# VincentStimper/normalizing-flows

Hardware: AMD Instinct MI355X
Metric: samples/sec + NLL (nats/dim), 32-layer RQ-NSF d=64 B=65536 (higher is better)
Workload: dtype f32; 1 GPU; BASELINE configs[1]: log_prob of 32 x [CoupledRQS(d=64, 2 blocks, 128 hidden, K=8, tail 3) + LULinearPermute(64)] + DiagGaussian, batch 65536 rows/GPU, N(0,I) inputs, sigma=0.01 perturbed seeded weights; rows_per_gpu=65536, global_rows=65536, layers=32, launch=hipGraph replay, parallelism=dp1

## Files before the change

include/nf_mi355x.h:

```cpp
#ifndef NF_MI355X_H
#define NF_MI355X_H

#include <stdint.h>

#ifdef __cplusplus
extern "C" {
#endif

typedef void *nf_stream_t;

enum { NF_OK = 0, NF_EIO = -5, NF_EFAULT = -14, NF_EINVAL = -22, NF_ERANGE = -34, NF_ENOTSUP = -95 };
enum { NF_F32 = 0, NF_F64 = 1 };
enum { NF_LD_WRITE = 0, NF_LD_ADD = 1, NF_LD_SUB = -1 };
enum { NF_TAILS_NONE = 0, NF_TAILS_LINEAR = 1, NF_TAILS_CIRCULAR = 2, NF_TAILS_FEATURE = 3  };
enum { NF_SCALE_EXP = 0, NF_SCALE_SIGMOID = 1, NF_SCALE_SIGMOID_INV = 2, NF_SCALE_NONE = 3 };
enum { NF_RQS_DENSITY = 0, NF_RQS_SAMPLE_IDENTITY = 1, NF_RQS_SAMPLE_TRANSFORM = 2 };

const char *nf_version(void);
const char *nf_strerror(int code);
int nf_mfma_clock_probe(void *out2_u64, void *sink_f32, int iters, nf_stream_t stream);
int nf_max_bins(void);
int nf_persistent_workgroups(void);

int nf_rqs_spline(const void *x, const void *w, int64_t ldw, const void *h, int64_t ldh, const void *d,
// ... 22 lines not shown
                        const int64_t *transform_idx, int nT, int64_t B, int D, int K, int tails,
                        double tail_bound, double min_bin_width, double min_bin_height, double min_derivative,
                        double wh_div, int mode, void *grad_x, void *grad_cond, void *grad_uw, void *grad_uh,
                        void *grad_ud, int dtype, nf_stream_t stream);

int nf_rqs_coupling_bwd_ft(const void *x, const void *grad_y, const void *grad_logdet, const void *cond,
                           const void *uw, const void *uh, const void *ud, const int64_t *identity_idx, int nI,
                           const int64_t *transform_idx, int nT, int64_t B, int D, int K, int tails,
                           double tail_bound, double min_bin_width, double min_bin_height, double min_derivative,
                           double wh_div, int mode, void *grad_x, void *grad_cond, void *grad_uw, void *grad_uh,
                           void *grad_ud, int dtype, const int32_t *tails_t, const void *bound_t,
                           const int32_t *tails_i, const void *bound_i, nf_stream_t stream);

int nf_rqs_coupling_bwd_ft_wave_fits(int nI, int nT);
int nf_rqs_coupling_bwd_ft_wave(const void *x, const void *grad_y, const void *grad_logdet, const void *cond,
                                const void *uw, const void *uh, const void *ud, const int64_t *identity_idx, int nI,
                                const int64_t *transform_idx, int nT, int64_t B, int D, int K, int tails,
                                double tail_bound, double min_bin_width, double min_bin_height, double min_derivative,
                                double wh_div, int mode, void *grad_x, void *grad_cond, void *grad_uw, void *grad_uh,
                                void *grad_ud, int dtype, const int32_t *tails_t, const void *bound_t,
                                const int32_t *tails_i, const void *bound_i, nf_stream_t stream);

int nf_rqs_fused_final_row(int K, int g, int rb, int rho);
int64_t nf_rqs_fused_pack_size(int nI, int nT, int hidden, int num_blocks, int K);
int nf_rqs_fused_pack(void *wpack, const void *w_init, const void *b_init, const void *const *w_blocks,
                      const void *const *b_blocks, const void *w_final, const void *b_final, const void *uw,
                      const void *uh, const void *ud, int nI, int nT, int hidden, int num_blocks, int K,
                      double tail_bound, double min_bin_width, double min_bin_height, double min_derivative,
                      nf_stream_t stream);
int nf_rqs_fused_pack_lu(void *wpack, int num_blocks, const int64_t *perm, const void *lower_entries,
                         const void *upper_entries, const void *unconstrained_upper_diag, const void *bias, int D,
                         double eps, int K, nf_stream_t stream);
int nf_rqs_fused(const void *x, void *y, void *logdet, const void *wpack, int mask_parity, int fuse_lu, int64_t B,
                 int D, int hidden, int num_blocks, int K, double tail_bound, double min_bin_width,
                 double min_bin_height, double min_derivative, int direction, int acc, nf_stream_t stream);
int nf_rqs_fused_chain(const void *x, void *y, void *logdet, const void *const *wpacks, const int *mask_parities,
                       int num_layers, int fuse_lu, int64_t B, int D, int hidden, int num_blocks, int K,
                       double tail_bound, double min_bin_width, double min_bin_height, double min_derivative,
                       int direction, int acc, nf_stream_t stream);
int nf_rqs_fused_small_batch(int enable);

int nf_rqs_fused_pack_final(void *wpack, const void *w_final, const void *b_final, const void *uw, const void *uh,
                            const void *ud, int hidden, int num_blocks, int K, double tail_bound, double min_bin_width,
                            double min_bin_height, double min_derivative, nf_stream_t stream);
int nf_rqs_fused_train_fwd(const void *x, const void *h2, void *y, void *logdet, void *cond_out, const void *wpack,
                           int mask_parity, int64_t B, int D, int hidden, int num_blocks, int K, double tail_bound,
// ... 333 lines not shown
```

normalizing-flows_amd/csrc/fused_common.hpp:

```cpp
#pragma once
#include "common.hpp"

namespace nf {

constexpr int F_MAX_LAYERS = 64;

typedef float f32x16 __attribute__((ext_vector_type(16)));
typedef float f32x4 __attribute__((ext_vector_type(4)));

constexpr int F_D = 64;
constexpr int F_NI = 32;
constexpr int F_H = 128;
constexpr int F_K = 8;
constexpr int F_M = 3 * F_K - 1;
constexpr int F_STAGE = 4096;
constexpr int F_TABW = 3 * (F_K + 1);
constexpr int F_HDR = 64;

struct FusedLayout {
    int nblk;
    int K = F_K;
    __host__ __device__ int ngroups() const { return K; }
    __host__ __device__ int nfinal() const { return 3 * K; }
    __host__ __device__ int tabw() const { return 3 * (K + 1); }
    __host__ __device__ int bias_final_floats() const { return 96 * K; }
    __host__ __device__ int small_floats() const { return 128 + 256 * nblk + bias_final_floats() + F_NI * tabw() + 128; }
    __host__ __device__ int off_bias_init() const { return 0; }
    __host__ __device__ int off_bias_hidden(int lin) const { return 128 + 128 * lin; }
    __host__ __device__ int off_bias_final() const { return 128 + 256 * nblk; }
    __host__ __device__ int off_tables() const { return off_bias_final() + bias_final_floats(); }
    __host__ __device__ int off_bias_lu(int dir) const { return off_tables() + F_NI * tabw() + 64 * dir; }
    __host__ __device__ int lu_stage(int dir) const { return 1 + 8 * nblk + nfinal() + dir; }
    __host__ __device__ int small_padded() const { return (small_floats() + 1023) / 1024 * 1024; }
    __host__ __device__ int off_stages() const { return F_HDR + small_padded(); }
    __host__ __device__ int nstages(bool lu) const { return 1 + 8 * nblk + nfinal() + (lu ? 1 : 0); }
    __host__ __device__ int64_t total_floats() const { return (int64_t)off_stages() + (int64_t)(nstages(false) + 2) * F_STAGE; }
};

template <int KB>
__host__ __device__ inline int final_row_k(int g, int rb, int rho) {
    constexpr int MP = 3 * KB, M = 3 * KB - 1, FPL = 16 / KB, GQ = KB / 4;
    const int q = rho >> 3, hh = (rho >> 2) & 1, r = rho & 3;
    const int v = 16 * rb + 4 * q + r;
    const int f = v / MP, prm = v % MP;
    if (prm >= M) return -1;
    const int tf = 8 * (g / GQ) + 4 * hh + (g % GQ) * FPL + f;
    return tf * M + prm;
}
__host__ __device__ inline int final_row(int g, int rb, int rho) { return final_row_k<F_K>(g, rb, rho); }

__host__ __device__ inline int final_bwd_row(int g, int v, int hq) {
    return v >= F_M ? -1 : (8 * (g >> 1) + 4 * (hq >> 1) + 2 * (g & 1) + (hq & 1)) * F_M + v;
}

__host__ __device__ inline int lu_out_col(int m, int rho) {
    const int q = rho >> 3, hh = (rho >> 2) & 1, r = rho & 3;
    return 16 * (2 * m + (q >> 1)) + 8 * hh + 4 * (q & 1) + r;
}
__host__ __device__ inline int lu_in_col(int s, int hk, int r4) { return 16 * (s >> 1) + 8 * hk + 4 * (s & 1) + r4; }

__device__ __forceinline__ float fexp(float x) { return __builtin_amdgcn_exp2f(x * 1.44269504088896340736f); }
__device__ __forceinline__ float flog(float x) { return __builtin_amdgcn_logf(x) * 0.69314718055994530942f; }
__device__ __forceinline__ float frcp(float x) { return __builtin_amdgcn_rcpf(x); }
__device__ __forceinline__ float fsqrt(float x) { return __builtin_amdgcn_sqrtf(x); }
__device__ __forceinline__ float fsoftplus(float x) {
    const float t = fexp(fminf(x, 20.0f));
    const float u = 1.0f + t;
    const float w = u - 1.0f;
    const float l1p = (w == 0.0f) ? t : flog(u) * (t * frcp(w));
    return x > 20.0f ? x : l1p;
}

// ... 68 lines not shown
    }
    float dl0 = p.edge_logit, dl1 = p.edge_logit;
#pragma unroll
    for (int k = 0; k < KB - 1; ++k) {
        dl0 = (bin == k + 1) ? prm[2 * KB + k] : dl0;
        dl1 = (bin == k) ? prm[2 * KB + k] : dl1;
    }
    const float d0 = p.min_d + fsoftplus(dl0), d1 = p.min_d + fsoftplus(dl1);
    float yy, ll;
    if (!INVERSE)
        rqs_eval_bin_fast<false>(x, slo, shi - slo, olo, ohi - olo, d0, d1, yy, ll);
    else
        rqs_eval_bin_fast<true>(x, olo, ohi - olo, slo, shi - slo, d0, d1, yy, ll);
    y = inside ? yy : x;
    lad = inside ? ll : 0.0f;
}

typedef float f32x2e __attribute__((ext_vector_type(2)));
typedef int i32x2e __attribute__((ext_vector_type(2)));
__device__ __forceinline__ f32x2e pk_fma(f32x2e a, f32x2e b, f32x2e c) { return __builtin_elementwise_fma(a, b, c); }
__device__ __forceinline__ f32x2e pk_rcp(f32x2e a) { return f32x2e{frcp(a[0]), frcp(a[1])}; }
__device__ __forceinline__ f32x2e pk_log(f32x2e a) { return f32x2e{flog(a[0]), flog(a[1])}; }
__device__ __forceinline__ f32x2e pk_bc(float a) { return f32x2e{a, a}; }

template <int N>
__device__ __forceinline__ void rqs_descend2(f32x2e x, const f32x2e (&s)[N + 1], const f32x2e (&o)[N + 1], const f32x2e (&d)[N + 1],
                                             f32x2e &slo, f32x2e &shi, f32x2e &olo, f32x2e &ohi, f32x2e &dl0, f32x2e &dl1) {
    if constexpr (N == 1) {
        slo = s[0]; shi = s[1]; olo = o[0]; ohi = o[1]; dl0 = d[0]; dl1 = d[1];
    } else {
        constexpr int H = N / 2;
        const i32x2e c = x >= s[H];
        f32x2e s2[H + 1], o2[H + 1], d2[H + 1];
#pragma unroll
        for (int i = 0; i <= H; ++i) {
            s2[i] = c ? s[H + i] : s[i];
            o2[i] = c ? o[H + i] : o[i];
            d2[i] = c ? d[H + i] : d[i];
        }
        rqs_descend2<H>(x, s2, o2, d2, slo, shi, olo, ohi, dl0, dl1);
    }
}

template <bool INVERSE>
__device__ __forceinline__ void rqs_eval_bin_fast2(f32x2e x, f32x2e cw, f32x2e bw, f32x2e ch, f32x2e bh, f32x2e d0, f32x2e d1,
                                                   f32x2e &y, f32x2e &lad) {
    const f32x2e delta = bh * pk_rcp(bw);
    const f32x2e dsum = d0 + d1 - 2.0f * delta;
    f32x2e theta, den;
    if (!INVERSE) {
        theta = (x - cw) * pk_rcp(bw);
        const f32x2e t1mt = theta * (1.0f - theta);
        const f32x2e num = bh * (delta * theta * theta + d0 * t1mt);
        den = delta + dsum * t1mt;
        y = ch + num * pk_rcp(den);
    } else {
        const f32x2e dy = x - ch;
        const f32x2e a = dy * dsum + bh * (delta - d0);
        const f32x2e b = bh * d0 - dy * dsum;
        const f32x2e c = -delta * dy;
        const f32x2e disc = b * b - 4.0f * a * c;
        theta = (2.0f * c) * pk_rcp(-b - f32x2e{fsqrt(disc[0]), fsqrt(disc[1])});
        y = theta * bw + cw;
        den = delta + dsum * (theta * (1.0f - theta));
    }
    const f32x2e omt = 1.0f - theta;
    const f32x2e dnum = delta * delta * (d1 * theta * theta + 2.0f * delta * (theta * omt) + d0 * omt * omt);
    const f32x2e l = pk_log(dnum) - 2.0f * pk_log(den);
    lad = INVERSE ? -l : l;
}

template <bool INVERSE, int KB = F_K>
__device__ __forceinline__ void rqs_regs2(const RqsParams<float> &p, float x0, float x1, const float (&prm0)[3 * KB],
                                          const float (&prm1)[3 * KB], float &y0, float &y1, float &lad0, float &lad1) {
    static_assert((KB & (KB - 1)) == 0, "binary descent");
    const f32x2e x = {x0, x1};
    const i32x2e inside = (x >= p.left) & (x <= p.right);
    f32x2e mw = {prm0[0], prm1[0]}, mh = {prm0[KB], prm1[KB]};
#pragma unroll
    for (int k = 1; k < KB; ++k) {
        mw = f32x2e{fmaxf(mw[0], prm0[k]), fmaxf(mw[1], prm1[k])};
        mh = f32x2e{fmaxf(mh[0], prm0[KB + k]), fmaxf(mh[1], prm1[KB + k])};
    }
    f32x2e pw[KB], ph[KB];
#pragma unroll
    for (int k = 0; k < KB; ++k) {
        const f32x2e aw = f32x2e{prm0[k], prm1[k]} - mw, ah = f32x2e{prm0[KB + k], prm1[KB + k]} - mh;
        const f32x2e ew = {__builtin_amdgcn_exp2f(aw[0]), __builtin_amdgcn_exp2f(aw[1])};
        const f32x2e eh = {__builtin_amdgcn_exp2f(ah[0]), __builtin_amdgcn_exp2f(ah[1])};
        pw[k] = k == 0 ? ew : pw[k - 1] + ew;
        ph[k] = k == 0 ? eh : ph[k - 1] + eh;
    }
    const f32x2e cw = ((p.right - p.left) * p.scale_w) * pk_rcp(pw[KB - 1]);
    const f32x2e ch = ((p.top - p.bottom) * p.scale_h) * pk_rcp(ph[KB - 1]);
    f32x2e kw[KB + 1], kh[KB + 1], dp[KB + 1];
    kw[0] = pk_bc(p.left);
    kh[0] = pk_bc(p.bottom);
    kw[KB] = pk_bc(p.right);
    kh[KB] = pk_bc(p.top);
    dp[0] = dp[KB] = pk_bc(p.edge_logit);
#pragma unroll
    for (int k = 1; k < KB; ++k) {
        kw[k] = pk_fma(pw[k - 1], cw, pk_bc(p.left + (p.right - p.left) * p.min_w * (float)k));
        kh[k] = pk_fma(ph[k - 1], ch, pk_bc(p.bottom + (p.top - p.bottom) * p.min_h * (float)k));
        dp[k] = f32x2e{prm0[2 * KB + k - 1], prm1[2 * KB + k - 1]};
    }
    f32x2e slo, shi, olo, ohi, dl0, dl1;
    if (!INVERSE)
        rqs_descend2<KB>(x, kw, kh, dp, slo, shi, olo, ohi, dl0, dl1);
    else
        rqs_descend2<KB>(x, kh, kw, dp, slo, shi, olo, ohi, dl0, dl1);
    const f32x2e d0 = p.min_d + f32x2e{fsoftplus(dl0[0]), fsoftplus(dl0[1])};
    const f32x2e d1 = p.min_d + f32x2e{fsoftplus(dl1[0]), fsoftplus(dl1[1])};
    f32x2e yy, ll;
    if (!INVERSE)
        rqs_eval_bin_fast2<false>(x, slo, shi - slo, olo, ohi - olo, d0, d1, yy, ll);
    else
        rqs_eval_bin_fast2<true>(x, olo, ohi - olo, slo, shi - slo, d0, d1, yy, ll);
    const f32x2e yr = inside ? yy : x;
    const f32x2e lr = inside ? ll : pk_bc(0.0f);
    y0 = yr[0]; y1 = yr[1]; lad0 = lr[0]; lad1 = lr[1];
}

template <int N>
__device__ __forceinline__ void rqs_descend1(float x, const float (&s)[N + 1], const float (&o)[N + 1], const float (&d)[N + 1],
                                             float &slo, float &shi, float &olo, float &ohi, float &dl0, float &dl1) {
    if constexpr (N == 1) {
        slo = s[0]; shi = s[1]; olo = o[0]; ohi = o[1]; dl0 = d[0]; dl1 = d[1];
    } else {
        constexpr int H = N / 2;
        const bool c = x >= s[H];
        float s2[H + 1], o2[H + 1], d2[H + 1];
#pragma unroll
        for (int i = 0; i <= H; ++i) {
            s2[i] = c ? s[H + i] : s[i];
            o2[i] = c ? o[H + i] : o[i];
            d2[i] = c ? d[H + i] : d[i];
        }
        rqs_descend1<H>(x, s2, o2, d2, slo, shi, olo, ohi, dl0, dl1);
    }
}
// ... 139 lines not shown
```

normalizing-flows_amd/csrc/rqs_fused.hip:

```cpp
#include "fused_common.hpp"

#ifndef NF_TRAIN_TEMPORAL_STORES
#define NF_TRAIN_STORE(ptr, val) __builtin_nontemporal_store((val), (ptr))
#else
#define NF_TRAIN_STORE(ptr, val) (*(ptr) = (val))
#endif

#ifdef NF_FUSED_SECONDARY
#define rqs_fused_kernel rqs_fused_kernel_nw4
#endif

namespace nf {

#ifndef NF_FUSED_SECONDARY
__global__ void pack_init_kernel(const float *__restrict__ W , const float *__restrict__ b, float *__restrict__ stage,
                                 float *__restrict__ bias_dst) {
    for (int i = blockIdx.x * blockDim.x + threadIdx.x; i < F_STAGE; i += gridDim.x * blockDim.x) {
        const int r4 = i & 3, lane = (i >> 2) & 63, s = (i >> 8) & 3, m = i >> 10;
        const int row = 32 * m + (lane & 31);
        const int k = 8 * s + 4 * (lane >> 5) + r4;
        stage[i] = W[row * F_NI + k];
    }
    for (int i = blockIdx.x * blockDim.x + threadIdx.x; i < 128; i += gridDim.x * blockDim.x) {
        const int reg = i & 15, hh = (i >> 4) & 1, m = i >> 5;
// ... 15 lines not shown
    }
}

template <int KB>
__global__ void pack_final_kernel(const float *__restrict__ W , const float *__restrict__ b,
                                  float *__restrict__ stages , float *__restrict__ bias_dst,
                                  float wh_scale) {
    constexpr int M = 3 * KB - 1;
    for (int i = blockIdx.x * blockDim.x + threadIdx.x; i < 3 * KB * F_STAGE; i += gridDim.x * blockDim.x) {
        const int r4 = i & 3, lane = (i >> 2) & 63, s = (i >> 8) & 15, st = i >> 12;
        const int g = st / 3, rb = st % 3;
        const int row = final_row_k<KB>(g, rb, lane & 31);
        const int k = 8 * s + 4 * (lane >> 5) + r4;
        const float sc = (row >= 0 && (row % M) < 2 * KB) ? wh_scale : 1.0f;
        stages[i] = row >= 0 ? W[row * F_H + k] * sc : 0.0f;
    }
    for (int i = blockIdx.x * blockDim.x + threadIdx.x; i < 96 * KB; i += gridDim.x * blockDim.x) {
        const int reg = i & 15, hh = (i >> 4) & 1, st = i >> 5;
        const int g = st / 3, rb = st % 3;
        const int row = final_row_k<KB>(g, rb, 8 * (reg >> 2) + 4 * hh + (reg & 3));
        const float sc = (row >= 0 && (row % M) < 2 * KB) ? wh_scale : 1.0f;
        bias_dst[i] = row >= 0 ? b[row] * sc : 0.0f;
    }
}

__global__ void pack_tables_kernel(const float *__restrict__ uw, const float *__restrict__ uh, const float *__restrict__ ud,
                                   float *__restrict__ tab, RqsParams<float> p) {
    const int j = blockIdx.x * blockDim.x + threadIdx.x;
    if (j >= F_NI) return;
    const int K = p.K;
    const float *wj = uw + j * K, *hj = uh + j * K, *dj = ud + j * (K - 1);
    auto wacc = [=](int k) { return wj[k]; };
    auto hacc = [=](int k) { return hj[k]; };
    auto dacc = [=](int k) { return dj[k]; };
    rqs_build_table<float>(p, wacc, hacc, dacc, tab + j * 3 * (K + 1));
}

__global__ void pack_header_kernel(float *__restrict__ hdr, int nblk) {
    if (threadIdx.x == 0 && blockIdx.x == 0) {
        hdr[0] = 355.0f;
        hdr[1] = (float)nblk;
        hdr[2] = 0.0f;
        hdr[3] = 0.0f;
    }
}

// ... 251 lines not shown
constexpr int F_DMA_WAVES = NF_DMA_WAVES < F_NW ? NF_DMA_WAVES : F_NW;
constexpr int F_THREADS = 64 * F_NW;
constexpr int F_ROWS = 32 * F_NW;

struct FlowArgs {
    const float *blob[F_MAX_LAYERS];
    unsigned long long parity;
    int nlayers;
    int ngroups;
};

template <int DIR, bool LU, int TRAIN = 0, int KB = F_K, int HB = 4>
__global__ void __launch_bounds__(F_THREADS, 2)
rqs_fused_kernel(const float *__restrict__ x, float *__restrict__ y, float *__restrict__ logdet, FlowArgs fa,
                 int64_t B, int nblk, RqsParams<float> p, int acc, const float *__restrict__ h_in = nullptr,
                 float *__restrict__ cond_out = nullptr, float unscale = 1.0f, float *__restrict__ act_out = nullptr,
                 float *__restrict__ xlu_out = nullptr) {
    extern __shared__ __attribute__((aligned(16))) float smem[];
    constexpr int LA = (HB == 4 && !(DIR == 0 && LU) && TRAIN == 0) ? 1 : 2;
    static_assert(KB == 4 || KB == 8 || KB == 16, "bins");
    static_assert(!TRAIN || (KB == F_K && DIR == 0 && (!LU || TRAIN == 2)),
                  "the training variants: 8 bins, density direction; the fused LU only with the whole-layer forward (TRAIN = 2)");
    static_assert(HB == 4 || ((HB == 2 || HB == 1) && !TRAIN), "hidden row-blocks");
    constexpr int MP = 3 * KB, FPL = 16 / KB, GQ = KB / 4, TABW = 3 * (KB + 1);
    FusedLayout lay;
    lay.nblk = nblk;
    lay.K = KB;
    float *ring = smem;
    float *stash = ring + 2 * F_STAGE;
    float *small2 = stash + F_NW * 32 * 64;
    const int small_pitch = lay.small_padded();
    const int tid = threadIdx.x, lane = tid & 63, hh = lane >> 5;
    const int wid = __builtin_amdgcn_readfirstlane(tid >> 6);
    const int64_t row = (int64_t)blockIdx.x * F_ROWS + wid * 32 + (lane & 31);
    const bool valid = row < B;
    const int nhid = 2 * nblk * HB;
    const int ngrp = TRAIN ? KB : fa.ngroups;
    const int nbase = 1 + nhid + 3 * ngrp;
    const int nstages = TRAIN == 1 ? 24 : nbase + (LU ? 1 : 0);
    const int total_stages = nstages * fa.nlayers;
    auto phys_base = [&](int b) -> int {
        if (HB == 4 || b == 0) return b;
        if (b <= nhid) return 1 + 4 * ((b - 1) / HB) + (b - 1) % HB;
        return 1 + 8 * nblk + (b - 1 - nhid);
    };
    auto phys = [&](int s) -> int {
        if (TRAIN == 1) return 1 + 8 * nblk + s;
        if (!LU) return phys_base(s);
        if (DIR == 0) return s == 0 ? lay.lu_stage(0) : phys_base(s - 1);
        return s < nbase ? phys_base(s) : lay.lu_stage(1);
    };
    float *st = stash + wid * 2048 + lane;

    int stage = 0;
    auto issue = [&](int gs) {
        constexpr int PPW = 16 / F_DMA_WAVES;
        if (wid >= F_DMA_WAVES) return;
        const int layer = gs / nstages, s = gs - layer * nstages;
        const float *src = fa.blob[layer] + lay.off_stages() + (size_t)phys(s) * F_STAGE + (wid * PPW) * 256 + lane * 4;
        float *dst = ring + (gs & 1) * F_STAGE + (wid * PPW) * 256;
#ifdef NF_BUILTIN_DMA
#pragma unroll
        for (int i = 0; i < PPW; ++i)
            __builtin_amdgcn_global_load_lds(src + i * 256, (__attribute__((address_space(3))) void *)(dst + i * 256), 16, 0, 0);
// ... 282 lines not shown
            st[s1 * 64] = y1;
            ld += l0;
            ld += l1;
        }
#endif
    };
    auto uncond_group = [&](int g) {
#ifdef NF_ABL_NOUNCOND
        return;
#endif
        const float *tabs = small + lay.off_tables();
#pragma unroll
        for (int e = 0; e < FPL; ++e) {
            const int r = FPL * (g % GQ) + e;
            const int c = 8 * (g / GQ) + 2 * r + par_i;
            const int f = 8 * (g / GQ) + 4 * hh + r;
            float yi, l;
            rqs_table_fast<false, KB>(p, st[c * 64], tabs + f * TABW, yi, l);
            st[c * 64] = yi;
            ld += l;
        }
    };
#ifdef NF_F32_SWPIPE
    static_assert(KB == F_K && HB == 4, "the software-pipelined order is written for 8 bins, 128 hidden units");
    {
        const float *bsrc = small + lay.off_bias_final() + hh * 16;
        f32x16 A0 = load_bias16(bsrc), A1 = load_bias16(bsrc + 32), A2 = load_bias16(bsrc + 64);
        mm128<false, 4, LA>(acquire(), lane, A0, H0, H1, H2, H3);
        mm128<false, 4, LA>(acquire(), lane, A1, H0, H1, H2, H3);
        mm128<false, 4, LA>(acquire(), lane, A2, H0, H1, H2, H3);
        extract(A0, A1, A2);
    }
    for (int g = 1; g < 8; ++g) {
        const float *bsrc = small + lay.off_bias_final() + (g * 3) * 32 + hh * 16;
        f32x16 A0 = load_bias16(bsrc), A1 = load_bias16(bsrc + 32), A2 = load_bias16(bsrc + 64);
        {
            const float *buf = acquire();
            mm128<false, 4, LA>(buf, lane, A0, H0, H1, H2, H3);
            element(g - 1, 0);
            NF_SCHED_PIPE();
        }
        {
            const float *buf = acquire();
            mm128<false, 4, LA>(buf, lane, A1, H0, H1, H2, H3);
            element(g - 1, 1);
            NF_SCHED_PIPE();
        }
        {
            const float *buf = acquire();
            mm128<false, 4, LA>(buf, lane, A2, H0, H1, H2, H3);
            if (DIR == 0) uncond_group(g - 1);
            NF_SCHED_PIPE();
        }
        extract(A0, A1, A2);
    }
    element(7, 0);
    element(7, 1);
    if (DIR == 0) uncond_group(7);
#else
    for (int g = 0; g < ngrp; ++g) {
        const float *bsrc = small + lay.off_bias_final() + (g * 3) * 32 + hh * 16;
        f32x16 A0 = load_bias16(bsrc), A1 = load_bias16(bsrc + 32), A2 = load_bias16(bsrc + 64);
        {
            const float *buf = acquire(g > 0 ? 14 : 0);
#ifndef NF_EXP_RELU_PER_USE
            if (g == 0) {
                if (nblk == 0) store_xlu();
                store_act(2 * nblk, H0, H1, H2, H3);
            }
#endif
            mm128<false, HB, LA>(buf, lane, A0, H0, H1, H2, H3);
        }
        mm128<false, HB, LA>(acquire(), lane, A1, H0, H1, H2, H3);
        mm128<false, HB, LA>(acquire(), lane, A2, H0, H1, H2, H3);
        extract(A0, A1, A2);
#ifdef NF_ABL_NOCOND
        if constexpr (false) {
#else
        if constexpr (TRAIN) {
#endif
#ifdef NF_TRAIN_DIRECT_STORES
            if (valid) {
// ... 122 lines not shown
        for (int64_t i = tid0; i < (int64_t)24 * F_STAGE; i += nth) {
            const int st = (int)(i >> 12), j = (int)(i & (F_STAGE - 1));
            const int u4 = j & 3, lane = (j >> 2) & 63, uq = (j >> 8) & 1, vv = j >> 9;
            const int row = final_bwd_row(st / 3, 8 * (st % 3) + vv, lane >> 4);
            a.wpad[i] = row >= 0 ? a.w_final[row * F_H + 16 * (4 * uq + u4) + (lane & 15)] : 0.0f;
        }
    }
    const int nbias = 128 + 128 * nlin + 768;
    for (int64_t i = tid0; i < nbias; i += nth) {
        const int reg = i & 15, hh = (i >> 4) & 1;
        float v;
        if (i < 128 + 128 * nlin) {
            const int blk = (int)(i >> 7), m = (int)((i >> 5) & 3);
            const float *b = blk == 0 ? a.b_init : a.b_blk[blk - 1];
            v = b[32 * m + 8 * (reg >> 2) + 4 * hh + (reg & 3)];
        } else {
            const int st = (int)((i - 128 - 128 * nlin) >> 5), g = st / 3, rb = st % 3;
            const int row = final_row(g, rb, 8 * (reg >> 2) + 4 * hh + (reg & 3));
            const float sc = (row >= 0 && (row % F_M) < 2 * F_K) ? wh_scale : 1.0f;
            v = row >= 0 ? a.b_final[row] * sc : 0.0f;
        }
        small[i] = v;
    }
    if (blockIdx.x == gridDim.x - 1) {
        const int j = threadIdx.x;
        if (j == 0) {
            blob[0] = 355.0f;
            blob[1] = (float)a.nblk;
            blob[2] = 0.0f;
            blob[3] = 0.0f;
        }
        if (j < F_NI) {
            const float *wj = a.uw + j * F_K, *hj = a.uh + j * F_K, *dj = a.ud + j * (F_K - 1);
            auto wacc = [=](int k) { return wj[k]; };
            auto hacc = [=](int k) { return hj[k]; };
            auto dacc = [=](int k) { return dj[k]; };
            rqs_build_table<float>(p, wacc, hacc, dacc, small + lay.off_tables() + j * F_TABW);
        }
    }
}

__global__ void pack_all_kernel(PackAllArgs a, float *__restrict__ blob, float wh_scale, RqsParams<float> p) {
    pack_all_body(a, blob, wh_scale, p);
}

__global__ void pack_all_multi_kernel(const void *const *__restrict__ table, int cols, int nblk, float wh_scale, RqsParams<float> p) {
// ... 8 lines not shown
        a.wfull = (float *)row[8]; a.wpad = (float *)row[9]; a.iidx = (const int64_t *)row[10];
        a.nblk = nblk;
        for (int l = 0; l < 2 * nblk; ++l) {
            a.w_blk[l] = (const float *)row[11 + l];
            a.b_blk[l] = (const float *)row[11 + 2 * nblk + l];
        }
    }
    __syncthreads();
    pack_all_body(a, blob, wh_scale, p);
}
#endif

}

using namespace nf;

static inline bool fused_bins_ok(int K) { return K == 4 || K == 8 || K == 16; }

template <bool LU>
static int train_fwd_launch(const void *x, void *xlu_out, void *y, void *logdet, void *cond_out, void *act_out, const FlowArgs &fa,
                            int64_t B, int hidden, int num_blocks, const RqsParams<float> &p, int acc, hipStream_t st) {
    FusedLayout lay;
    lay.nblk = num_blocks;
    const size_t lds = (size_t)(2 * F_STAGE + F_NW * 32 * 64 + lay.small_padded() + F_NW * 1536) * sizeof(float);
    if (lds > 160 * 1024) return NF_ENOTSUP;
    static LdsOptIn opted = {};
    if (opt_in_lds(reinterpret_cast<const void *>(&rqs_fused_kernel<0, LU, 2>), lds, opted) != NF_OK) return NF_ENOTSUP;
    const int grid = (int)((B + F_ROWS - 1) / F_ROWS);
    hipLaunchKernelGGL((rqs_fused_kernel<0, LU, 2>), dim3(grid), dim3(F_THREADS), lds, st, (const float *)x, (float *)y,
                       (float *)logdet, fa, B, num_blocks, p, acc, (const float *)nullptr, (float *)cond_out,
                       (float)(sqrt((double)hidden) / 1.4426950408889634), (float *)act_out, (float *)xlu_out);
    NF_CHECK_LAUNCH();
    return NF_OK;
}

#ifdef NF_FUSED_SECONDARY
extern "C" int nf_rqs_fused_train_fwd_nw4_(int lu, const void *x, void *xlu_out, void *y, void *logdet, void *cond_out, void *act_out,
                                           const void *fa, int64_t B, int hidden, int num_blocks, const void *p, int acc,
                                           nf_stream_t stream) {
    const FlowArgs &f = *static_cast<const FlowArgs *>(fa);
    const RqsParams<float> &pp = *static_cast<const RqsParams<float> *>(p);
    return lu ? train_fwd_launch<true>(x, xlu_out, y, logdet, cond_out, act_out, f, B, hidden, num_blocks, pp, acc, (hipStream_t)stream)
              : train_fwd_launch<false>(x, xlu_out, y, logdet, cond_out, act_out, f, B, hidden, num_blocks, pp, acc, (hipStream_t)stream);
}
#endif

#ifndef NF_FUSED_SECONDARY
// ... 93 lines not shown
    if (g_small_batch && B <= NF_FUSED_SMALL_ROWS)
        return nf_rqs_fused_train_fwd_nw4_(1, x, xlu_out, y, logdet, cond_out, act_out, &fa, B, hidden, num_blocks, &p, acc, stream);
    return train_fwd_launch<true>(x, xlu_out, y, logdet, cond_out, act_out, fa, B, hidden, num_blocks, p, acc, (hipStream_t)stream);
}

extern "C" int nf_lu_pack_train_multi(const void *table, int n_layers, int num_blocks, int D, double eps, nf_stream_t stream) {
    if (D != F_D || num_blocks < 0 || num_blocks > 16) return NF_ENOTSUP;
    if (n_layers < 0 || n_layers > 65535) return NF_EINVAL;
    if (n_layers == 0) return NF_OK;
    if (!table) return NF_EFAULT;
    const size_t lds = (size_t)3 * F_D * F_D * sizeof(double) + F_D * sizeof(int) + 64;
    static LdsOptIn opted = {};
    if (opt_in_lds(reinterpret_cast<const void *>(&pack_lu_train_multi_kernel), lds, opted) != NF_OK) return NF_ENOTSUP;
    hipLaunchKernelGGL(pack_lu_train_multi_kernel, dim3(n_layers), dim3(256), lds, (hipStream_t)stream, (const void *const *)table,
                       (float)eps, num_blocks);
    NF_CHECK_LAUNCH();
    return NF_OK;
}

extern "C" int nf_rqs_fused_final_row(int K, int g, int rb, int rho) {
    if (!fused_bins_ok(K)) return NF_ENOTSUP;
    if (g < 0 || g >= K || rb < 0 || rb > 2 || rho < 0 || rho > 31) return NF_EINVAL;
    return K == 4 ? final_row_k<4>(g, rb, rho) : (K == 8 ? final_row_k<8>(g, rb, rho) : final_row_k<16>(g, rb, rho));
}

extern "C" int64_t nf_rqs_fused_pack_size(int nI, int nT, int hidden, int num_blocks, int K) {
    if (nI != F_NI || nT != F_NI || hidden != F_H || !fused_bins_ok(K) || num_blocks < 0 || num_blocks > 16) return NF_ENOTSUP;
    FusedLayout lay;
    lay.nblk = num_blocks;
    lay.K = K;
    return lay.total_floats() * (int64_t)sizeof(float);
}

extern "C" int nf_rqs_fused_pack(void *wpack, const void *w_init, const void *b_init, const void *const *w_blocks,
                                 const void *const *b_blocks, const void *w_final, const void *b_final, const void *uw,
                                 const void *uh, const void *ud, int nI, int nT, int hidden, int num_blocks, int K,
                                 double tail_bound, double min_bin_width, double min_bin_height, double min_derivative,
                                 nf_stream_t stream) {
    if (nI != F_NI || nT != F_NI || hidden != F_H || !fused_bins_ok(K) || num_blocks < 0 || num_blocks > 16) return NF_ENOTSUP;
    if (!wpack || !w_init || !b_init || !w_final || !b_final || !uw || !uh || !ud) return NF_EFAULT;
    if (num_blocks > 0 && (!w_blocks || !b_blocks)) return NF_EFAULT;
    if (min_bin_width * K > 1.0 || min_bin_height * K > 1.0) return NF_EINVAL;
    hipStream_t st = (hipStream_t)stream;
    FusedLayout lay;
    lay.nblk = num_blocks;
    lay.K = K;
    float *blob = (float *)wpack;
    float *small = blob + F_HDR;
    float *stages = blob + lay.off_stages();
    hipLaunchKernelGGL(pack_header_kernel, dim3(1), dim3(64), 0, st, blob, num_blocks);
    hipLaunchKernelGGL(pack_init_kernel, dim3(16), dim3(256), 0, st, (const float *)w_init, (const float *)b_init, stages,
                       small + lay.off_bias_init());
    for (int l = 0; l < 2 * num_blocks; ++l) {
        if (!w_blocks[l] || !b_blocks[l]) return NF_EFAULT;
        hipLaunchKernelGGL(pack_hidden_kernel, dim3(64), dim3(256), 0, st, (const float *)w_blocks[l],
                           (const float *)b_blocks[l], stages + (size_t)(1 + 4 * l) * F_STAGE,
                           small + lay.off_bias_hidden(l));
    }
#define NF_PACK_FINAL(KB)                                                                                            \
    hipLaunchKernelGGL(pack_final_kernel<KB>, dim3(48 * KB), dim3(256), 0, st, (const float *)w_final,                   \
                       (const float *)b_final, stages + (size_t)(1 + 8 * num_blocks) * F_STAGE,                          \
                       small + lay.off_bias_final(), (float)(1.4426950408889634 / sqrt((double)hidden)))
    if (K == 4) NF_PACK_FINAL(4);
    else if (K == 8) NF_PACK_FINAL(8);
    else NF_PACK_FINAL(16);
#undef NF_PACK_FINAL
    auto p = make_rqs_params<float>(K, NF_TAILS_LINEAR, tail_bound, 0, 1, 0, 1, min_bin_width, min_bin_height,
                                    min_derivative, 1.0);
    hipLaunchKernelGGL(pack_tables_kernel, dim3(1), dim3(64), 0, st, (const float *)uw, (const float *)uh,
                       (const float *)ud, small + lay.off_tables(), p);
    NF_CHECK_LAUNCH();
    return NF_OK;
}

extern "C" int nf_rqs_fused_pack_final(void *wpack, const void *w_final, const void *b_final, const void *uw, const void *uh,
                                       const void *ud, int hidden, int num_blocks, int K, double tail_bound,
                                       double min_bin_width, double min_bin_height, double min_derivative, nf_stream_t stream) {
    if (hidden != F_H || K != F_K || num_blocks < 0 || num_blocks > 16) return NF_ENOTSUP;
    if (!wpack || !w_final || !b_final || !uw || !uh || !ud) return NF_EFAULT;
    if (min_bin_width * K > 1.0 || min_bin_height * K > 1.0) return NF_EINVAL;
    hipStream_t st = (hipStream_t)stream;
    FusedLayout lay;
    lay.nblk = num_blocks;
    float *blob = (float *)wpack;
    float *small = blob + F_HDR;
    float *stages = blob + lay.off_stages();
    auto p = make_rqs_params<float>(K, NF_TAILS_LINEAR, tail_bound, 0, 1, 0, 1, min_bin_width, min_bin_height,
                                    min_derivative, 1.0);
    hipLaunchKernelGGL(pack_final_all_kernel, dim3(384), dim3(256), 0, st, (const float *)w_final, (const float *)b_final,
// ... 121 lines not shown
        return nf_rqs_fused_chain_nw4_(x, y, logdet, &fa, B, hidden, num_blocks, K, &p, direction, fuse_lu, acc, stream);
    return chain_dispatch(x, y, logdet, fa, B, hidden, num_blocks, K, p, direction, fuse_lu, acc, (hipStream_t)stream);
}

extern "C" int nf_rqs_fused_train_fwd(const void *x, const void *h2, void *y, void *logdet, void *cond_out, const void *wpack,
                                      int mask_parity, int64_t B, int D, int hidden, int num_blocks, int K, double tail_bound,
                                      double min_bin_width, double min_bin_height, double min_derivative, int acc,
                                      nf_stream_t stream) {
    if (D != F_D || hidden != F_H || K != F_K || num_blocks < 0 || num_blocks > 16) return NF_ENOTSUP;
    if (B < 0 || (mask_parity != 0 && mask_parity != 1) || acc < NF_LD_SUB || acc > NF_LD_ADD) return NF_EINVAL;
    if (B == 0) return NF_OK;
    if (!x || !h2 || !y || !logdet || !cond_out || !wpack) return NF_EFAULT;
    if (nf_misaligned16(x, h2, y, cond_out, wpack)) return NF_EINVAL;
    FlowArgs fa;
    fa.parity = mask_parity ? 1ull : 0ull;
    fa.nlayers = 1;
    fa.ngroups = F_K;
    for (int l = 0; l < F_MAX_LAYERS; ++l) fa.blob[l] = nullptr;
    fa.blob[0] = (const float *)wpack;
    FusedLayout lay;
    lay.nblk = num_blocks;
    auto p = make_rqs_params<float>(K, NF_TAILS_LINEAR, tail_bound, 0, 1, 0, 1, min_bin_width, min_bin_height,
                                    min_derivative, sqrt((double)hidden));
    const size_t lds = (size_t)(2 * F_STAGE + F_NW * 32 * 64 + lay.small_padded() + F_NW * 1536) * sizeof(float);
    if (lds > 160 * 1024) return NF_ENOTSUP;
    static LdsOptIn opted = {};
    if (opt_in_lds(reinterpret_cast<const void *>(&rqs_fused_kernel<0, false, true>), lds, opted) != NF_OK) return NF_ENOTSUP;
    const int grid = (int)((B + F_ROWS - 1) / F_ROWS);
    hipLaunchKernelGGL((rqs_fused_kernel<0, false, true>), dim3(grid), dim3(F_THREADS), lds, (hipStream_t)stream, (const float *)x,
                       (float *)y, (float *)logdet, fa, B, num_blocks, p, acc, (const float *)h2, (float *)cond_out,
                       (float)(sqrt((double)hidden) / 1.4426950408889634));
    NF_CHECK_LAUNCH();
    return NF_OK;
}

extern "C" int nf_rqs_fused(const void *x, void *y, void *logdet, const void *wpack, int mask_parity, int fuse_lu,
                            int64_t B, int D, int hidden, int num_blocks, int K, double tail_bound, double min_bin_width,
                            double min_bin_height, double min_derivative, int direction, int acc, nf_stream_t stream) {
    const void *packs[1] = {wpack};
    const int par[1] = {mask_parity};
    if (!wpack) return NF_EFAULT;
    return nf_rqs_fused_chain(x, y, logdet, packs, par, 1, fuse_lu, B, D, hidden, num_blocks, K, tail_bound, min_bin_width,
                              min_bin_height, min_derivative, direction, acc, stream);
}
#endif
```

Baseline: 11.99 million samples/s.

## Pack compact final-layer weights using softmax shift invariance to cut MFMA stages

Softmax is invariant to a shift, so the final linear layer is repacked as weight differences against the first width and height logit of each feature, and one boundary derivative row is dropped. This takes each feature from 24 output rows to 21, which reduces the number of final-section row-block stages streamed and multiplied per layer (42 rows per feature pair instead of 48). The spline max reduction is rewritten with v_max3 over a known zero first logit. Refined reciprocals, one Newton step each, are enabled on this path, adding extra ALU work. Pack size, LDS layout and the pack kernels all grow a compact section. Training paths keep the legacy layout.

```diff
diff --git a/include/nf_mi355x.h b/include/nf_mi355x.h
--- a/include/nf_mi355x.h
+++ b/include/nf_mi355x.h
@@ -68,6 +68,8 @@
                                 const int32_t *tails_i, const void *bound_i, nf_stream_t stream);
 
 int nf_rqs_fused_final_row(int K, int g, int rb, int rho);
+#define NF_RQS_COMPACT_DIFF (1 << 16)
+int nf_rqs_fused_compact_row(int K, int rb, int rho);
 int64_t nf_rqs_fused_pack_size(int nI, int nT, int hidden, int num_blocks, int K);
 int nf_rqs_fused_pack(void *wpack, const void *w_init, const void *b_init, const void *const *w_blocks,
                       const void *const *b_blocks, const void *w_final, const void *b_final, const void *uw,
diff --git a/normalizing-flows_amd/csrc/fused_common.hpp b/normalizing-flows_amd/csrc/fused_common.hpp
--- a/normalizing-flows_amd/csrc/fused_common.hpp
+++ b/normalizing-flows_amd/csrc/fused_common.hpp
@@ -25,16 +25,21 @@
     __host__ __device__ int tabw() const { return 3 * (K + 1); }
     __host__ __device__ int bias_final_floats() const { return 96 * K; }
     __host__ __device__ int small_floats() const { return 128 + 256 * nblk + bias_final_floats() + F_NI * tabw() + 128; }
+    __host__ __device__ int ncompact() const { return K == 8 ? 21 : 0; }
+    __host__ __device__ int bias_compact_floats() const { return 32 * ncompact(); }
+    __host__ __device__ int off_bias_compact() const { return small_floats(); }
+    __host__ __device__ int compact_stage(int rb) const { return 1 + 8 * nblk + nfinal() + 2 + rb; }
     __host__ __device__ int off_bias_init() const { return 0; }
     __host__ __device__ int off_bias_hidden(int lin) const { return 128 + 128 * lin; }
     __host__ __device__ int off_bias_final() const { return 128 + 256 * nblk; }
     __host__ __device__ int off_tables() const { return off_bias_final() + bias_final_floats(); }
     __host__ __device__ int off_bias_lu(int dir) const { return off_tables() + F_NI * tabw() + 64 * dir; }
     __host__ __device__ int lu_stage(int dir) const { return 1 + 8 * nblk + nfinal() + dir; }
-    __host__ __device__ int small_padded() const { return (small_floats() + 1023) / 1024 * 1024; }
+    __host__ __device__ int small_padded() const { return (small_floats() + bias_compact_floats() + 1023) / 1024 * 1024; }
+    __host__ __device__ int small_padded_legacy() const { return (small_floats() + 1023) / 1024 * 1024; }
     __host__ __device__ int off_stages() const { return F_HDR + small_padded(); }
     __host__ __device__ int nstages(bool lu) const { return 1 + 8 * nblk + nfinal() + (lu ? 1 : 0); }
-    __host__ __device__ int64_t total_floats() const { return (int64_t)off_stages() + (int64_t)(nstages(false) + 2) * F_STAGE; }
+    __host__ __device__ int64_t total_floats() const { return (int64_t)off_stages() + (int64_t)(nstages(false) + 2 + ncompact()) * F_STAGE; }
 };
 
 template <int KB>
@@ -48,6 +53,25 @@
     return tf * M + prm;
 }
 __host__ __device__ inline int final_row(int g, int rb, int rho) { return final_row_k<F_K>(g, rb, rho); }
+
+constexpr int F_COMPACT_DIFF = 1 << 16;
+constexpr int F_NCOMPACT = 21;
+__host__ __device__ inline int compact_row(int rb, int rho) {
+    const int q = rho >> 3, hh = (rho >> 2) & 1, r = rho & 3;
+    const int v = 16 * rb + 4 * q + r;
+    const int j = v / 42, f = (v % 42) / 21, c = v % 21;
+    const int tf = 8 * (j >> 1) + 4 * hh + 2 * (j & 1) + f;
+    if (c < 7) return (tf * F_M + 1 + c) | F_COMPACT_DIFF;
+    if (c < 14) return (tf * F_M + F_K + 1 + (c - 7)) | F_COMPACT_DIFF;
+    return tf * F_M + 2 * F_K + (c - 14);
+}
+template <class At>
+__host__ __device__ inline float compact_value(int rb, int rho, float wh_scale, At at) {
+    const int cr = compact_row(rb, rho), row = cr & (F_COMPACT_DIFF - 1);
+    if (!(cr & F_COMPACT_DIFF)) return at(row);
+    const int prm = row % F_M, row0 = row - prm + (prm < F_K ? 0 : F_K);
+    return (at(row) - at(row0)) * wh_scale;
+}
 
 __host__ __device__ inline int final_bwd_row(int g, int v, int hq) {
     return v >= F_M ? -1 : (8 * (g >> 1) + 4 * (hq >> 1) + 2 * (g & 1) + (hq & 1)) * F_M + v;
@@ -162,6 +186,12 @@
 __device__ __forceinline__ f32x2e pk_rcp(f32x2e a) { return f32x2e{frcp(a[0]), frcp(a[1])}; }
 __device__ __forceinline__ f32x2e pk_log(f32x2e a) { return f32x2e{flog(a[0]), flog(a[1])}; }
 __device__ __forceinline__ f32x2e pk_bc(float a) { return f32x2e{a, a}; }
+template <bool FINE>
+__device__ __forceinline__ f32x2e pk_rcp_t(f32x2e a) {
+    f32x2e r = pk_rcp(a);
+    if constexpr (FINE) r = pk_fma(r, pk_fma(-a, r, pk_bc(1.0f)), r);
+    return r;
+}
 
 template <int N>
 __device__ __forceinline__ void rqs_descend2(f32x2e x, const f32x2e (&s)[N + 1], const f32x2e (&o)[N + 1], const f32x2e (&d)[N + 1],
@@ -182,25 +212,25 @@
     }
 }
 
-template <bool INVERSE>
+template <bool INVERSE, bool FINE = false>
 __device__ __forceinline__ void rqs_eval_bin_fast2(f32x2e x, f32x2e cw, f32x2e bw, f32x2e ch, f32x2e bh, f32x2e d0, f32x2e d1,
                                                    f32x2e &y, f32x2e &lad) {
-    const f32x2e delta = bh * pk_rcp(bw);
+    const f32x2e delta = bh * pk_rcp_t<FINE>(bw);
     const f32x2e dsum = d0 + d1 - 2.0f * delta;
     f32x2e theta, den;
     if (!INVERSE) {
-        theta = (x - cw) * pk_rcp(bw);
+        theta = (x - cw) * pk_rcp_t<FINE>(bw);
         const f32x2e t1mt = theta * (1.0f - theta);
         const f32x2e num = bh * (delta * theta * theta + d0 * t1mt);
         den = delta + dsum * t1mt;
-        y = ch + num * pk_rcp(den);
+        y = ch + num * pk_rcp_t<FINE>(den);
     } else {
         const f32x2e dy = x - ch;
         const f32x2e a = dy * dsum + bh * (delta - d0);
         const f32x2e b = bh * d0 - dy * dsum;
         const f32x2e c = -delta * dy;
         const f32x2e disc = b * b - 4.0f * a * c;
-        theta = (2.0f * c) * pk_rcp(-b - f32x2e{fsqrt(disc[0]), fsqrt(disc[1])});
+        theta = (2.0f * c) * pk_rcp_t<FINE>(-b - f32x2e{fsqrt(disc[0]), fsqrt(disc[1])});
         y = theta * bw + cw;
         den = delta + dsum * (theta * (1.0f - theta));
     }
@@ -210,17 +240,41 @@
     lad = INVERSE ? -l : l;
 }
 
-template <bool INVERSE, int KB = F_K>
+__device__ __forceinline__ float fmax3_raw(float a, float b, float c) {
+    float r;
+    asm("v_max3_f32 %0, %1, %2, %3" : "=v"(r) : "v"(a), "v"(b), "v"(c));
+    return r;
+}
+__device__ __forceinline__ float fmax3_raw0(float b, float c) {
+    float r;
+    asm("v_max3_f32 %0, 0, %1, %2" : "=v"(r) : "v"(b), "v"(c));
+    return r;
+}
+__device__ __forceinline__ float fmax_raw(float a, float b) {
+    float r;
+    asm("v_max_f32 %0, %1, %2" : "=v"(r) : "v"(a), "v"(b));
+    return r;
+}
+
+template <bool INVERSE, int KB = F_K, bool Z0 = false>
 __device__ __forceinline__ void rqs_regs2(const RqsParams<float> &p, float x0, float x1, const float (&prm0)[3 * KB],
                                           const float (&prm1)[3 * KB], float &y0, float &y1, float &lad0, float &lad1) {
     static_assert((KB & (KB - 1)) == 0, "binary descent");
     const f32x2e x = {x0, x1};
     const i32x2e inside = (x >= p.left) & (x <= p.right);
     f32x2e mw = {prm0[0], prm1[0]}, mh = {prm0[KB], prm1[KB]};
-#pragma unroll
-    for (int k = 1; k < KB; ++k) {
-        mw = f32x2e{fmaxf(mw[0], prm0[k]), fmaxf(mw[1], prm1[k])};
-        mh = f32x2e{fmaxf(mh[0], prm0[KB + k]), fmaxf(mh[1], prm1[KB + k])};
+    if constexpr (Z0) {
+        static_assert(KB == 8, "the compact final section");
+#define NF_MAX8(q, o) fmax_raw(fmax3_raw(fmax3_raw(fmax3_raw0(q[o + 1], q[o + 2]), q[o + 3], q[o + 4]), q[o + 5], q[o + 6]), q[o + 7])
+        mw = f32x2e{NF_MAX8(prm0, 0), NF_MAX8(prm1, 0)};
+        mh = f32x2e{NF_MAX8(prm0, KB), NF_MAX8(prm1, KB)};
+#undef NF_MAX8
+    } else {
+#pragma unroll
+        for (int k = 1; k < KB; ++k) {
+            mw = f32x2e{fmaxf(mw[0], prm0[k]), fmaxf(mw[1], prm1[k])};
+            mh = f32x2e{fmaxf(mh[0], prm0[KB + k]), fmaxf(mh[1], prm1[KB + k])};
+        }
     }
     f32x2e pw[KB], ph[KB];
 #pragma unroll
@@ -254,9 +308,9 @@
     const f32x2e d1 = p.min_d + f32x2e{fsoftplus(dl1[0]), fsoftplus(dl1[1])};
     f32x2e yy, ll;
     if (!INVERSE)
-        rqs_eval_bin_fast2<false>(x, slo, shi - slo, olo, ohi - olo, d0, d1, yy, ll);
-    else
-        rqs_eval_bin_fast2<true>(x, olo, ohi - olo, slo, shi - slo, d0, d1, yy, ll);
+        rqs_eval_bin_fast2<false, Z0>(x, slo, shi - slo, olo, ohi - olo, d0, d1, yy, ll);
+    else
+        rqs_eval_bin_fast2<true, Z0>(x, olo, ohi - olo, slo, shi - slo, d0, d1, yy, ll);
     const f32x2e yr = inside ? yy : x;
     const f32x2e lr = inside ? ll : pk_bc(0.0f);
     y0 = yr[0]; y1 = yr[1]; lad0 = lr[0]; lad1 = lr[1];
diff --git a/normalizing-flows_amd/csrc/rqs_fused.hip b/normalizing-flows_amd/csrc/rqs_fused.hip
--- a/normalizing-flows_amd/csrc/rqs_fused.hip
+++ b/normalizing-flows_amd/csrc/rqs_fused.hip
@@ -1,4 +1,5 @@
 #include "fused_common.hpp"
+#include <type_traits>
 
 #ifndef NF_TRAIN_TEMPORAL_STORES
 #define NF_TRAIN_STORE(ptr, val) __builtin_nontemporal_store((val), (ptr))
@@ -61,6 +62,24 @@
         const float sc = (row >= 0 && (row % M) < 2 * KB) ? wh_scale : 1.0f;
         bias_dst[i] = row >= 0 ? b[row] * sc : 0.0f;
     }
+}
+
+__device__ __forceinline__ void pack_compact_body(const float *__restrict__ W , const float *__restrict__ b,
+                                                  float *__restrict__ stages , float *__restrict__ bias_dst,
+                                                  float wh_scale, int64_t tid0, int64_t nth) {
+    for (int64_t i = tid0; i < (int64_t)F_NCOMPACT * F_STAGE; i += nth) {
+        const int r4 = i & 3, lane = (i >> 2) & 63, s = (i >> 8) & 15, rb = (int)(i >> 12);
+        const int k = 8 * s + 4 * (lane >> 5) + r4;
+        stages[i] = compact_value(rb, lane & 31, wh_scale, [=](int row) { return W[row * F_H + k]; });
+    }
+    for (int64_t i = tid0; i < 32 * F_NCOMPACT; i += nth) {
+        const int reg = i & 15, hh = (i >> 4) & 1, rb = (int)(i >> 5);
+        bias_dst[i] = compact_value(rb, 8 * (reg >> 2) + 4 * hh + (reg & 3), wh_scale, [=](int row) { return b[row]; });
+    }
+}
+__global__ void pack_compact_kernel(const float *__restrict__ W, const float *__restrict__ b, float *__restrict__ stages,
+                                    float *__restrict__ bias_dst, float wh_scale) {
+    pack_compact_body(W, b, stages, bias_dst, wh_scale, (int64_t)blockIdx.x * blockDim.x + threadIdx.x, (int64_t)gridDim.x * blockDim.x);
 }
 
 __global__ void pack_tables_kernel(const float *__restrict__ uw, const float *__restrict__ uh, const float *__restrict__ ud,
@@ -358,6 +377,7 @@
     static_assert(!TRAIN || (KB == F_K && DIR == 0 && (!LU || TRAIN == 2)),
                   "the training variants: 8 bins, density direction; the fused LU only with the whole-layer forward (TRAIN = 2)");
     static_assert(HB == 4 || ((HB == 2 || HB == 1) && !TRAIN), "hidden row-blocks");
+    constexpr bool COMPACT = KB == 8 && TRAIN == 0;
     constexpr int MP = 3 * KB, FPL = 16 / KB, GQ = KB / 4, TABW = 3 * (KB + 1);
     FusedLayout lay;
     lay.nblk = nblk;
@@ -365,17 +385,20 @@
     float *ring = smem;
     float *stash = ring + 2 * F_STAGE;
     float *small2 = stash + F_NW * 32 * 64;
-    const int small_pitch = lay.small_padded();
+    const int small_pitch = TRAIN ? lay.small_padded_legacy() : lay.small_padded();
     const int tid = threadIdx.x, lane = tid & 63, hh = lane >> 5;
     const int wid = __builtin_amdgcn_readfirstlane(tid >> 6);
     const int64_t row = (int64_t)blockIdx.x * F_ROWS + wid * 32 + (lane & 31);
     const bool valid = row < B;
     const int nhid = 2 * nblk * HB;
     const int ngrp = TRAIN ? KB : fa.ngroups;
-    const int nbase = 1 + nhid + 3 * ngrp;
+    const int nbase = 1 + nhid + (COMPACT ? (42 * ngrp + 15) >> 4 : 3 * ngrp);
     const int nstages = TRAIN == 1 ? 24 : nbase + (LU ? 1 : 0);
     const int total_stages = nstages * fa.nlayers;
     auto phys_base = [&](int b) -> int {
+        if constexpr (COMPACT) {
+            if (b > nhid) return lay.compact_stage(b - 1 - nhid);
+        }
         if (HB == 4 || b == 0) return b;
         if (b <= nhid) return 1 + 4 * ((b - 1) / HB) + (b - 1) % HB;
         return 1 + 8 * nblk + (b - 1 - nhid);
@@ -704,6 +727,7 @@
         }
     };
 #ifdef NF_F32_SWPIPE
+    static_assert(!COMPACT, "the software-pipelined order streams the 24 legacy stages");
     static_assert(KB == F_K && HB == 4, "the software-pipelined order is written for 8 bins, 128 hidden units");
     {
         const float *bsrc = small + lay.off_bias_final() + hh * 16;
@@ -740,6 +764,56 @@
     element(7, 1);
     if (DIR == 0) uncond_group(7);
 #else
+    if constexpr (COMPACT) {
+        const float *bfin = small + lay.off_bias_compact() + hh * 16;
+        f32x16 C = {};
+        auto pair = [&](auto jc) __attribute__((always_inline)) {
+            constexpr int J = decltype(jc)::value;
+            constexpr int S0 = 42 * J, RN = (S0 + 15) / 16, RE = (S0 + 42 + 15) / 16, NNEW = RE - RN;
+            static_assert(NNEW == 2 || NNEW == 3, "row-blocks per pair");
+            f32x16 A0 = load_bias16(bfin + RN * 32), A1 = load_bias16(bfin + (RN + 1) * 32), A2 = A1;
+            mm128<false, HB, LA>(acquire(), lane, A0, H0, H1, H2, H3);
+            mm128<false, HB, LA>(acquire(), lane, A1, H0, H1, H2, H3);
+            if constexpr (NNEW == 3) {
+                A2 = load_bias16(bfin + (RN + 2) * 32);
+                mm128<false, HB, LA>(acquire(), lane, A2, H0, H1, H2, H3);
+            }
+            auto val = [&](int slot) -> float {
+                const int rb = slot >> 4, e = slot & 15;
+                return rb < RN ? C[e] : (rb == RN ? A0[e] : (rb == RN + 1 ? A1[e] : A2[e]));
+            };
+            float p0[MP], p1[MP];
+#pragma unroll
+            for (int v = 0; v < MP; ++v) {
+                const int c = v < KB ? v - 1 : v - 2;
+                const bool zero = v == 0 || v == KB || v == MP - 1;
+                p0[v] = zero ? 0.0f : val(S0 + c);
+                p1[v] = zero ? 0.0f : val(S0 + 21 + c);
+            }
+            C = NNEW == 3 ? A2 : A1;
+#ifdef NF_ABL_NOEPI
+#pragma unroll
+            for (int v = 0; v < MP; ++v) asm volatile("" ::"v"(p0[v]), "v"(p1[v]));
+#else
+            const int s0 = 8 * (J / 2) + 4 * (J % 2) + par_t, s1 = s0 + 2;
+            float y0, y1, l0, l1;
+            rqs_regs2<DIR == 1, KB, true>(p, st[s0 * 64], st[s1 * 64], p0, p1, y0, y1, l0, l1);
+            st[s0 * 64] = y0;
+            st[s1 * 64] = y1;
+            ld += l0;
+            ld += l1;
+#endif
+            if (DIR == 0) uncond_group(J);
+        };
+        pair(std::integral_constant<int, 0>{});
+        if (ngrp > 1) pair(std::integral_constant<int, 1>{});
+        if (ngrp > 2) pair(std::integral_constant<int, 2>{});
+        if (ngrp > 3) pair(std::integral_constant<int, 3>{});
+        if (ngrp > 4) pair(std::integral_constant<int, 4>{});
+        if (ngrp > 5) pair(std::integral_constant<int, 5>{});
+        if (ngrp > 6) pair(std::integral_constant<int, 6>{});
+        if (ngrp > 7) pair(std::integral_constant<int, 7>{});
+    } else
     for (int g = 0; g < ngrp; ++g) {
         const float *bsrc = small + lay.off_bias_final() + (g * 3) * 32 + hh * 16;
         f32x16 A0 = load_bias16(bsrc), A1 = load_bias16(bsrc + 32), A2 = load_bias16(bsrc + 64);
@@ -908,6 +982,8 @@
         }
         small[i] = v;
     }
+    pack_compact_body(a.w_final, a.b_final, stages + (size_t)lay.compact_stage(0) * F_STAGE, small + lay.off_bias_compact(), wh_scale,
+                      tid0, nth);
     if (blockIdx.x == gridDim.x - 1) {
         const int j = threadIdx.x;
         if (j == 0) {
@@ -962,7 +1038,7 @@
                             int64_t B, int hidden, int num_blocks, const RqsParams<float> &p, int acc, hipStream_t st) {
     FusedLayout lay;
     lay.nblk = num_blocks;
-    const size_t lds = (size_t)(2 * F_STAGE + F_NW * 32 * 64 + lay.small_padded() + F_NW * 1536) * sizeof(float);
+    const size_t lds = (size_t)(2 * F_STAGE + F_NW * 32 * 64 + lay.small_padded_legacy() + F_NW * 1536) * sizeof(float);
     if (lds > 160 * 1024) return NF_ENOTSUP;
     static LdsOptIn opted = {};
     if (opt_in_lds(reinterpret_cast<const void *>(&rqs_fused_kernel<0, LU, 2>), lds, opted) != NF_OK) return NF_ENOTSUP;
@@ -1102,6 +1178,12 @@
     if (!fused_bins_ok(K)) return NF_ENOTSUP;
     if (g < 0 || g >= K || rb < 0 || rb > 2 || rho < 0 || rho > 31) return NF_EINVAL;
     return K == 4 ? final_row_k<4>(g, rb, rho) : (K == 8 ? final_row_k<8>(g, rb, rho) : final_row_k<16>(g, rb, rho));
+}
+
+extern "C" int nf_rqs_fused_compact_row(int K, int rb, int rho) {
+    if (K != 8) return NF_ENOTSUP;
+    if (rb < 0 || rb >= F_NCOMPACT || rho < 0 || rho > 31) return NF_EINVAL;
+    return compact_row(rb, rho);
 }
 
 extern "C" int64_t nf_rqs_fused_pack_size(int nI, int nT, int hidden, int num_blocks, int K) {
@@ -1145,6 +1227,10 @@
     else if (K == 8) NF_PACK_FINAL(8);
     else NF_PACK_FINAL(16);
 #undef NF_PACK_FINAL
+    if (K == 8)
+        hipLaunchKernelGGL(pack_compact_kernel, dim3(21 * 16), dim3(256), 0, st, (const float *)w_final, (const float *)b_final,
+                           stages + (size_t)lay.compact_stage(0) * F_STAGE, small + lay.off_bias_compact(),
+                           (float)(1.4426950408889634 / sqrt((double)hidden)));
     auto p = make_rqs_params<float>(K, NF_TAILS_LINEAR, tail_bound, 0, 1, 0, 1, min_bin_width, min_bin_height,
                                     min_derivative, 1.0);
     hipLaunchKernelGGL(pack_tables_kernel, dim3(1), dim3(64), 0, st, (const float *)uw, (const float *)uh,
@@ -1312,7 +1398,7 @@
     lay.nblk = num_blocks;
     auto p = make_rqs_params<float>(K, NF_TAILS_LINEAR, tail_bound, 0, 1, 0, 1, min_bin_width, min_bin_height,
                                     min_derivative, sqrt((double)hidden));
-    const size_t lds = (size_t)(2 * F_STAGE + F_NW * 32 * 64 + lay.small_padded() + F_NW * 1536) * sizeof(float);
+    const size_t lds = (size_t)(2 * F_STAGE + F_NW * 32 * 64 + lay.small_padded_legacy() + F_NW * 1536) * sizeof(float);
     if (lds > 160 * 1024) return NF_ENOTSUP;
     static LdsOptIn opted = {};
     if (opt_in_lds(reinterpret_cast<const void *>(&rqs_fused_kernel<0, false, true>), lds, opted) != NF_OK) return NF_ENOTSUP;
```

Result: faster. 12.79 million samples/s, median of 6 (+6.7%).
